# zcash-hackworks/bn

Measured on AMD Instinct MI355X. Metric: BN254 optimal-ate pairings/sec (bit-exact vs ref), higher is better.
Workload: dtype u32; 1 GPU; 2^16 independent pairings per step on 1 MI355X (BASELINE.json configs[1]); pairings_per_gpu=65536, inputs=r*G1 / s*G2 (Jacobian, z != 1) resident in HBM, parallelism=dp1 (sharded, no collective), mapping=1, cus=256, pairings_per_launch=65536

## Files before the change

### bn_amd/csrc/bn254_constants.hpp

```cpp
#pragma once
#include <stdint.h>
#ifndef BN254_CONSTANT
#define BN254_CONSTANT constexpr
#endif
namespace bn254 { namespace k {
constexpr int W = 29, N = 9;
BN254_CONSTANT uint32_t MASK = 0x1fffffffu;
BN254_CONSTANT uint32_t Q[9] = {0x187cfd47u, 0x010460b6u, 0x1c72a34fu, 0x02d522d0u, 0x1585d978u, 0x02db40c0u, 0x00a6e141u, 0x0e5c2634u, 0x0030644eu};
BN254_CONSTANT uint32_t QINV = 0x04866389u;
BN254_CONSTANT uint32_t FE_MU = 0xa948e8c4u;
BN254_CONSTANT uint32_t FE_MU24 = 0x00a948e8u;
BN254_CONSTANT uint32_t ONE[9] = {0x157ccc21u, 0x141c2758u, 0x185230d3u, 0x014c0419u, 0x0aa36fb9u, 0x1d4240ceu, 0x11d54c07u, 0x052ac7a8u, 0x000dc836u};
BN254_CONSTANT uint32_t C_IN[9] = {0x13349ca1u, 0x1a5d84a8u, 0x0a3e5cacu, 0x100249e0u, 0x12b951e8u, 0x0e92d304u, 0x14cb95b3u, 0x041b9d3du, 0x00058003u};
BN254_CONSTANT uint32_t C_OUT[9] = {0x058f0d9du, 0x1aea1c6eu, 0x11c2cf74u, 0x11d651ebu, 0x1462c0a7u, 0x11b7bc3cu, 0x1cbd99bau, 0x183340fbu, 0x000e0a77u};
BN254_CONSTANT uint32_t RAW_ONE[9] = {0x00000001u, 0x00000000u, 0x00000000u, 0x00000000u, 0x00000000u, 0x00000000u, 0x00000000u, 0x00000000u, 0x00000000u};
BN254_CONSTANT uint32_t TWO_INV[9] = {0x16fce4b4u, 0x0a904407u, 0x0a626a11u, 0x12109375u, 0x1014a498u, 0x100ec0c7u, 0x093e16a4u, 0x09c376eeu, 0x001f1642u};
BN254_CONSTANT uint32_t G2_B[2][9] = {{0x0b489658u, 0x00cfd255u, 0x0fdb9a77u, 0x02ce89f7u, 0x0033a0d4u, 0x1a768545u, 0x06ee3ddcu, 0x106a7dc1u, 0x0019316bu}, {0x1b9fece0u, 0x07ecccd1u, 0x1069f1c7u, 0x0cdf64f3u, 0x0154cbe1u, 0x0dd22ac0u, 0x06eba4e8u, 0x1929a235u, 0x00283739u}};
BN254_CONSTANT uint32_t G2_3B[2][9] = {{0x095cc5c1u, 0x016b1649u, 0x13202c16u, 0x05967b15u, 0x0b150904u, 0x0c884f0eu, 0x1423d855u, 0x02e3530fu, 0x001b2ff4u}, {0x01e5cc12u, 0x15bda508u, 0x18588eb7u, 0x00f3e938u, 0x18f2b0b4u, 0x03bffebeu, 0x13752c37u, 0x0ec49a37u, 0x0017dd10u}};
BN254_CONSTANT uint32_t ISO_T2[9] = {0x1e3bec37u, 0x007b2046u, 0x19d0ea1fu, 0x1acb991fu, 0x13795f5du, 0x1055c3f5u, 0x15c8f72cu, 0x101310f5u, 0x002bf6bau};
BN254_CONSTANT uint32_t ISO_T3[9] = {0x1af1f8a3u, 0x00cd9858u, 0x1dce6a34u, 0x142e620au, 0x1bc0c667u, 0x0ae94d20u, 0x0db9310bu, 0x12572b72u, 0x000405e6u};
BN254_CONSTANT uint32_t FROB6_C1[4][2][9] = {
    {{0x157ccc21u, 0x141c2758u, 0x185230d3u, 0x014c0419u, 0x0aa36fb9u, 0x1d4240ceu, 0x11d54c07u, 0x052ac7a8u, 0x000dc836u}, {0x00000000u, 0x00000000u, 0x00000000u, 0x00000000u, 0x00000000u, 0x00000000u, 0x00000000u, 0x00000000u, 0x00000000u}},
    {{0x04a59190u, 0x06f504d9u, 0x0bf870bbu, 0x171ffd5cu, 0x1ac4d17du, 0x04be36d5u, 0x0bceec27u, 0x1a83a513u, 0x002492b3u}, {0x11142ef1u, 0x0b31acc7u, 0x1d5818bcu, 0x180afc17u, 0x1a63177eu, 0x15765b3bu, 0x118f742eu, 0x063a509au, 0x00135e4eu}},
    {{0x18ccb791u, 0x175b1c3au, 0x0b83d6e2u, 0x0e8ed071u, 0x1282bee2u, 0x04220e84u, 0x1fe4017fu, 0x15084d4au, 0x00169119u}, {0x00000000u, 0x00000000u, 0x00000000u, 0x00000000u, 0x00000000u, 0x00000000u, 0x00000000u, 0x00000000u, 0x00000000u}},
// ... 27 lines not shown
BN254_CONSTANT uint32_t TWIST_MUL_BY_Q_X[2][9] = {{0x04a59190u, 0x06f504d9u, 0x0bf870bbu, 0x171ffd5cu, 0x1ac4d17du, 0x04be36d5u, 0x0bceec27u, 0x1a83a513u, 0x002492b3u}, {0x11142ef1u, 0x0b31acc7u, 0x1d5818bcu, 0x180afc17u, 0x1a63177eu, 0x15765b3bu, 0x118f742eu, 0x063a509au, 0x00135e4eu}};
BN254_CONSTANT uint32_t TWIST_MUL_BY_Q_Y[2][9] = {{0x1b1f0678u, 0x0373fb06u, 0x13170fbdu, 0x185d74b7u, 0x0241131fu, 0x16e18435u, 0x1ef3b6ceu, 0x01f06f02u, 0x001d46bdu}, {0x19a647d5u, 0x19fdefabu, 0x1d925d1au, 0x0d1f6c5fu, 0x08ac6cc5u, 0x1fa5621au, 0x134f06feu, 0x09a72816u, 0x0015871du}};
BN254_CONSTANT uint64_t ATE_LOOP_LOW64 = 0x9d797039be763ba8ull;
BN254_CONSTANT uint64_t BN_U = 0x44e992b44a6909f1ull;
constexpr int BN_U_NAF_LEN = 63;
BN254_CONSTANT int8_t BN_U_NAF[63] = {1, 0, 0, 0, -1, 0, 0, 0, 0, 1, 0, 1, 0, 0, 0, 0, 1, 0, 0, 1, 0, -1, 0, 1, 0, 1, 0, 1, 0, 0, 1, 0, 0, 0, 1, 0, -1, 0, -1, 0, -1, 0, 1, 0, 1, 0, 0, -1, 0, 1, 0, 1, 0, -1, 0, 0, 1, 0, 1, 0, 0, 0, 1};
constexpr int EXP_SLOTS = 9;
constexpr int EXP_STEPS = 63;
BN254_CONSTANT int32_t EXP_SCHED[63] = {64, 1, 1, 1, 131, 195, 1, 1, 1, 1, 1, 39, 1, 1, 1, 1, 1, 1, 5, 1, 7, 1, 1, 1, 39, 1, 1, 1, 39, 1, 1, 1, 1, 1, 1, 1, 1, 7, 1, 1, 1, 7, 1, 1, 1, 1, 1, 5, 1, 1, 1, 1, 7, 1, 1, 1, 1, 37, 1, 1, 1, 1, 16389};
constexpr int FE_STEPS = 204;
BN254_CONSTANT int32_t FE_PROG[204] = {256, 64, 1, 1, 1, 131, 195, 1, 1, 1, 1, 1, 39, 1, 1, 1, 1, 1, 1, 5, 1, 7, 1, 1, 1, 39, 1, 1, 1, 39, 1, 1, 1, 1, 1, 1, 1, 1, 7, 1, 1, 1, 7, 1, 1, 1, 1, 1, 5, 1, 1, 1, 1, 7, 1, 1, 1, 1, 37, 1, 1, 1, 1, 16389, 321, 395, 64, 1, 1, 1, 131, 195, 1, 1, 1, 1, 1, 39, 1, 1, 1, 1, 1, 1, 5, 1, 7, 1, 1, 1, 39, 1, 1, 1, 39, 1, 1, 1, 1, 1, 1, 1, 1, 7, 1, 1, 1, 7, 1, 1, 1, 1, 1, 5, 1, 1, 1, 1, 7, 1, 1, 1, 1, 37, 1, 1, 1, 1, 16837, 1, 64, 1, 1, 1, 131, 195, 1, 1, 1, 1, 1, 39, 1, 1, 1, 1, 1, 1, 5, 1, 7, 1, 1, 1, 39, 1, 1, 1, 39, 1, 1, 1, 1, 1, 1, 1, 1, 7, 1, 1, 1, 7, 1, 1, 1, 1, 1, 5, 1, 1, 1, 1, 7, 1, 1, 1, 1, 37, 1, 1, 1, 1, 5, 14, 556, 586, 8206, 392, 41984, 460, 57344, 334, 74792, 10};
constexpr int ATE_NAF_LEN = 66;
BN254_CONSTANT int8_t ATE_NAF[66] = {0, 0, 0, 1, 0, 1, 0, -1, 0, 0, -1, 0, 0, 0, 1, 0, 0, -1, 0, -1, 0, 0, 0, 1, 0, -1, 0, 0, 0, 0, -1, 0, 0, 1, 0, -1, 0, 0, 1, 0, 0, 0, 0, 0, -1, 0, 0, -1, 0, 1, 0, -1, 0, 0, 0, -1, 0, -1, 0, 0, 0, 1, 0, -1, 0, 1};
BN254_CONSTANT int32_t Q30[9] = {0x187cfd47, 0x3082305b, 0x071ca8d3, 0x205aa45a, 0x01585d97, 0x0116da06, 0x1a029b85, 0x139cb84c, 0x00003064};
BN254_CONSTANT uint32_t QINV30 = 0x1b799c77u;
BN254_CONSTANT uint32_t C_R3[9] = {0x0e2312b2u, 0x16c05ca2u, 0x0bc84389u, 0x1cdf310bu, 0x11adafddu, 0x032e568eu, 0x1d6ae48cu, 0x10d4cd1fu, 0x0026c2d2u};
BN254_CONSTANT uint32_t C_RAW_IN[9] = {0x059bac10u, 0x0d1503a3u, 0x018016b8u, 0x10ab0ca8u, 0x02632639u, 0x02c0169fu, 0x169bfd53u, 0x11869d4cu, 0x002a11a6u};
BN254_CONSTANT uint32_t C_RAW_HI[9] = {0x0ff8e86au, 0x07c648f0u, 0x0d256c51u, 0x0e144bb5u, 0x0fe5cb16u, 0x0e4726c0u, 0x07f5c538u, 0x0f6c68ccu, 0x00043c5bu};
BN254_CONSTANT uint32_t Q32[8] = {0xd87cfd47u, 0x3c208c16u, 0x6871ca8du, 0x97816a91u, 0x8181585du, 0xb85045b6u, 0xe131a029u, 0x30644e72u};
BN254_CONSTANT uint32_t QINV256[8] = {0x1b799c77u, 0x782df87du, 0xe1359536u, 0x6121829au, 0xe7cc257fu, 0x2750342fu, 0x6e777394u, 0x0a85dd48u};
BN254_CONSTANT uint64_t R_MINUS_1[4] = {0x43e1f593f0000000ull, 0x2833e84879b97091ull, 0xb85045b68181585dull, 0x30644e72e131a029ull};
BN254_CONSTANT uint32_t G1_B[9] = {0x00766463u, 0x1c54760au, 0x08f6927au, 0x03e40c4du, 0x1fea4f2bu, 0x17c6c26au, 0x157fe417u, 0x0f8056f9u, 0x002958a2u};
BN254_CONSTANT uint64_t Q_MINUS_2[4] = {0x3c208c16d87cfd45ull, 0x97816a916871ca8dull, 0xb85045b68181585dull, 0x30644e72e131a029ull};
BN254_CONSTANT uint32_t H2C_C2[9] = {0x01801893u, 0x16741cafu, 0x1210393du, 0x10c48f5bu, 0x057134dfu, 0x12cc7ff9u, 0x1768ca9cu, 0x0498af45u, 0x00114e0cu};
BN254_CONSTANT uint32_t H2C_C3[9] = {0x1b4a814fu, 0x1d686287u, 0x16a42cbau, 0x0bac1e79u, 0x013fb16cu, 0x1d850693u, 0x1eba05b6u, 0x0c9dae1eu, 0x001b5818u};
BN254_CONSTANT uint32_t H2C_C4[9] = {0x068a0e4bu, 0x171eba7cu, 0x0b55234fu, 0x150690b3u, 0x0ed0a792u, 0x1ff392cau, 0x026922c2u, 0x109d85a1u, 0x002768ebu};
BN254_CONSTANT uint32_t H2C_G2_C1[2][9] = {{0x00c56279u, 0x14ebf9aeu, 0x082dcb4au, 0x041a8e11u, 0x0ad7108du, 0x17b8c613u, 0x18c389e4u, 0x15954569u, 0x0026f9a1u}, {0x1b9fece0u, 0x07ecccd1u, 0x1069f1c7u, 0x0cdf64f3u, 0x0154cbe1u, 0x0dd22ac0u, 0x06eba4e8u, 0x1929a235u, 0x00283739u}};
BN254_CONSTANT uint32_t H2C_G2_C3[2][9] = {{0x1ac12654u, 0x18b51d52u, 0x02b71328u, 0x0f302745u, 0x18dae6dfu, 0x1ec740f3u, 0x0ad8391fu, 0x1e701b16u, 0x002bf9c5u}, {0x1b8c55e3u, 0x07029597u, 0x09a398b3u, 0x06a5295fu, 0x152a0cd2u, 0x1080d518u, 0x1295607fu, 0x1129d51au, 0x00151bebu}};
BN254_CONSTANT uint32_t H2C_G2_C4[2][9] = {{0x1a9d7742u, 0x1b78c9dau, 0x18a8378fu, 0x1586dd8au, 0x1c979cdeu, 0x1b6acebcu, 0x159e5ffbu, 0x15469a85u, 0x002cd11au}, {0x017a140eu, 0x0ccd05abu, 0x0dad5994u, 0x148069b2u, 0x09454dc3u, 0x089e4881u, 0x1813914cu, 0x05d61ecbu, 0x002b29a5u}};
BN254_CONSTANT uint32_t GLV_BETA[9] = {0x0a337995u, 0x158d1d23u, 0x189c9b98u, 0x12fa4e45u, 0x185faadcu, 0x0176f16du, 0x0eed93bau, 0x14291140u, 0x000c0afeu};
BN254_CONSTANT uint32_t GLV_G1[3] = {0xc7e0b3d7u, 0xd91d232eu, 0x00000002u};
// ... 17 lines not shown
```

### bn_amd/csrc/fe.hpp

```cpp
#pragma once
#include <stdint.h>

#if defined(BN_HOSTSIM)
#define BN_FN inline
#define BN_LEAF inline
#define BN_LEAF_MUL inline
#define BN_LEAF_RED inline
#define BN_COARSE inline
#define BN_OUTER inline
#define BN254_CONSTANT constexpr
#define BN_COMPILER_FENCE() ((void)0)
#else
#include <hip/hip_runtime.h>
#define BN_FN __device__ __forceinline__
#define BN_LEAF __device__ __noinline__ inline
#ifdef BN_INLINE_ALL
#define BN_LEAF_MUL __device__ __forceinline__
#define BN_LEAF_RED __device__ __forceinline__
#define BN_COARSE __device__ __forceinline__
#else
#define BN_LEAF_MUL BN_LEAF
#define BN_LEAF_RED BN_LEAF
#define BN_COARSE __device__ __noinline__ inline
#endif
// ... 883 lines not shown
    uint32_t u = 1, v = 0, q = 0, r = 1, f = f0, g = g0;
#pragma unroll 1
    for (int i = 0; i < 30; ++i) {
        uint32_t mask1 = (uint32_t)(zeta >> 31);
        uint32_t mask2 = 0u - (g & 1u);
        uint32_t x = (f ^ mask1) - mask1, y = (u ^ mask1) - mask1, z = (v ^ mask1) - mask1;
        g += x & mask2; q += y & mask2; r += z & mask2;
        mask1 &= mask2;
        zeta = (int32_t)((uint32_t)zeta ^ mask1) - 1;
        f += g & mask1; u += q & mask1; v += r & mask1;
        g >>= 1; u <<= 1; v <<= 1;
    }
    tu = (int32_t)u; tv = (int32_t)v; tq = (int32_t)q; tr = (int32_t)r;
    return zeta;
}
BN_FN void divsteps_update_de(Signed30 &d, Signed30 &e, int32_t u, int32_t v, int32_t q, int32_t r) {
    const int32_t M30 = 0x3fffffff;
    int32_t sd = d.v[8] >> 31, se = e.v[8] >> 31;
    int32_t md = (u & sd) + (v & se), me = (q & sd) + (r & se);
    int32_t di = d.v[0], ei = e.v[0];
    int64_t cd = (int64_t)u * di + (int64_t)v * ei, ce = (int64_t)q * di + (int64_t)r * ei;
    md -= (int32_t)((k::QINV30 * (uint32_t)cd + (uint32_t)md) & (uint32_t)M30);
    me -= (int32_t)((k::QINV30 * (uint32_t)ce + (uint32_t)me) & (uint32_t)M30);
    cd += (int64_t)k::Q30[0] * md;
    ce += (int64_t)k::Q30[0] * me;
    cd >>= 30; ce >>= 30;
#pragma unroll
    for (int i = 1; i < 9; ++i) {
        di = d.v[i]; ei = e.v[i];
        cd += (int64_t)u * di + (int64_t)v * ei + (int64_t)k::Q30[i] * md;
// ... 18 lines not shown
    }
    f.v[8] = (int32_t)cf; g.v[8] = (int32_t)cg;
}
BN_FN Fe fe_inverse_body(const Fe &a_in) {
    BN_REQUIRE(a_in.lb <= 2 && a_in.vb <= 8 && !a_in.sg, "fe_inverse input");
    uint32_t w[8];
    fe_pack_u32x8(fe_canonical(fe_mul(a_in, fe_const(k::ONE))), w);
    Signed30 f, g, d, e;
#pragma unroll
    for (int i = 0; i < 9; ++i) {
        int bit = 30 * i, wi = bit >> 5, sh = bit & 31;
        uint64_t two = (uint64_t)w[wi] | (wi + 1 < 8 ? ((uint64_t)w[wi + 1] << 32) : 0);
        g.v[i] = (int32_t)((uint32_t)(two >> sh) & 0x3fffffffu);
        f.v[i] = k::Q30[i];
        d.v[i] = 0;
        e.v[i] = i == 0 ? 1 : 0;
    }
    int32_t zeta = -1;
#pragma unroll 1
    for (int it = 0; it < 20; ++it) {
        int32_t tu, tv, tq, tr;
        zeta = divsteps_30(zeta, (uint32_t)f.v[0], (uint32_t)g.v[0], tu, tv, tq, tr);
        divsteps_update_de(d, e, tu, tv, tq, tr);
        divsteps_update_fg(f, g, tu, tv, tq, tr);
    }
    const int32_t M30 = 0x3fffffff;
    int32_t r[9];
    int32_t cond_add = d.v[8] >> 31, cond_neg = f.v[8] >> 31;
#pragma unroll
    for (int i = 0; i < 9; ++i) { int32_t t = d.v[i] + (k::Q30[i] & cond_add); r[i] = (t ^ cond_neg) - cond_neg; }
#pragma unroll
    for (int i = 0; i < 8; ++i) { r[i + 1] += r[i] >> 30; r[i] &= M30; }
    cond_add = r[8] >> 31;
#pragma unroll
    for (int i = 0; i < 9; ++i) r[i] += k::Q30[i] & cond_add;
#pragma unroll
    for (int i = 0; i < 8; ++i) { r[i + 1] += r[i] >> 30; r[i] &= M30; }
#pragma unroll
    for (int j = 0; j < 8; ++j) {
        int bit = 32 * j, li = bit / 30, sh = bit - 30 * li;
        uint64_t vv = (uint64_t)(uint32_t)r[li] >> sh;
        if (li + 1 < 9) vv |= (uint64_t)(uint32_t)r[li + 1] << (30 - sh);
        w[j] = (uint32_t)vv;
    }
    return fe_mul(fe_unpack_u32x8(w), fe_const(k::C_R3));
}
BN_LEAF1(fe_inverse, fe_inverse_body)

}
```

### bn_amd/csrc/fe_asm.hpp

```cpp
#pragma once
namespace bn254 {
BN_FN Fe fe_mul_asm(const Fe &a, const Fe &b) {
    uint64_t acc;
    uint32_t m[9];
    Fe r;
    asm("v_mad_u64_u32 %0, vcc, %1, %2, 0" : "=&v"(acc) : "v"(a.l[0]), "v"(b.l[0]) : "vcc");
    m[0] = ((uint32_t)acc * k::QINV) & MASK29; acc += (uint64_t)m[0] * k::Q[0]; acc >>= 29;
    asm("v_mad_u64_u32 %0, vcc, %1, %2, %0\n\tv_mad_u64_u32 %0, vcc, %3, %4, %0\n\tv_mad_u64_u32 %0, vcc, %5, %6, %0" : "+v"(acc) : "v"(a.l[0]), "v"(b.l[1]), "v"(a.l[1]), "v"(b.l[0]), "v"(m[0]), "s"(k::Q[1]) : "vcc");
    m[1] = ((uint32_t)acc * k::QINV) & MASK29; acc += (uint64_t)m[1] * k::Q[0]; acc >>= 29;
    asm("v_mad_u64_u32 %0, vcc, %1, %2, %0\n\tv_mad_u64_u32 %0, vcc, %3, %4, %0\n\tv_mad_u64_u32 %0, vcc, %5, %6, %0\n\tv_mad_u64_u32 %0, vcc, %7, %8, %0\n\tv_mad_u64_u32 %0, vcc, %9, %10, %0" : "+v"(acc) : "v"(a.l[0]), "v"(b.l[2]), "v"(a.l[1]), "v"(b.l[1]), "v"(a.l[2]), "v"(b.l[0]), "v"(m[0]), "s"(k::Q[2]), "v"(m[1]), "s"(k::Q[1]) : "vcc");
    m[2] = ((uint32_t)acc * k::QINV) & MASK29; acc += (uint64_t)m[2] * k::Q[0]; acc >>= 29;
    asm("v_mad_u64_u32 %0, vcc, %1, %2, %0\n\tv_mad_u64_u32 %0, vcc, %3, %4, %0\n\tv_mad_u64_u32 %0, vcc, %5, %6, %0\n\tv_mad_u64_u32 %0, vcc, %7, %8, %0\n\tv_mad_u64_u32 %0, vcc, %9, %10, %0\n\tv_mad_u64_u32 %0, vcc, %11, %12, %0\n\tv_mad_u64_u32 %0, vcc, %13, %14, %0" : "+v"(acc) : "v"(a.l[0]), "v"(b.l[3]), "v"(a.l[1]), "v"(b.l[2]), "v"(a.l[2]), "v"(b.l[1]), "v"(a.l[3]), "v"(b.l[0]), "v"(m[0]), "s"(k::Q[3]), "v"(m[1]), "s"(k::Q[2]), "v"(m[2]), "s"(k::Q[1]) : "vcc");
    m[3] = ((uint32_t)acc * k::QINV) & MASK29; acc += (uint64_t)m[3] * k::Q[0]; acc >>= 29;
    asm("v_mad_u64_u32 %0, vcc, %1, %2, %0\n\tv_mad_u64_u32 %0, vcc, %3, %4, %0\n\tv_mad_u64_u32 %0, vcc, %5, %6, %0\n\tv_mad_u64_u32 %0, vcc, %7, %8, %0\n\tv_mad_u64_u32 %0, vcc, %9, %10, %0\n\tv_mad_u64_u32 %0, vcc, %11, %12, %0\n\tv_mad_u64_u32 %0, vcc, %13, %14, %0\n\tv_mad_u64_u32 %0, vcc, %15, %16, %0\n\tv_mad_u64_u32 %0, vcc, %17, %18, %0" : "+v"(acc) : "v"(a.l[0]), "v"(b.l[4]), "v"(a.l[1]), "v"(b.l[3]), "v"(a.l[2]), "v"(b.l[2]), "v"(a.l[3]), "v"(b.l[1]), "v"(a.l[4]), "v"(b.l[0]), "v"(m[0]), "s"(k::Q[4]), "v"(m[1]), "s"(k::Q[3]), "v"(m[2]), "s"(k::Q[2]), "v"(m[3]), "s"(k::Q[1]) : "vcc");
    m[4] = ((uint32_t)acc * k::QINV) & MASK29; acc += (uint64_t)m[4] * k::Q[0]; acc >>= 29;
    asm("v_mad_u64_u32 %0, vcc, %1, %2, %0\n\tv_mad_u64_u32 %0, vcc, %3, %4, %0\n\tv_mad_u64_u32 %0, vcc, %5, %6, %0\n\tv_mad_u64_u32 %0, vcc, %7, %8, %0\n\tv_mad_u64_u32 %0, vcc, %9, %10, %0\n\tv_mad_u64_u32 %0, vcc, %11, %12, %0\n\tv_mad_u64_u32 %0, vcc, %13, %14, %0\n\tv_mad_u64_u32 %0, vcc, %15, %16, %0\n\tv_mad_u64_u32 %0, vcc, %17, %18, %0\n\tv_mad_u64_u32 %0, vcc, %19, %20, %0\n\tv_mad_u64_u32 %0, vcc, %21, %22, %0" : "+v"(acc) : "v"(a.l[0]), "v"(b.l[5]), "v"(a.l[1]), "v"(b.l[4]), "v"(a.l[2]), "v"(b.l[3]), "v"(a.l[3]), "v"(b.l[2]), "v"(a.l[4]), "v"(b.l[1]), "v"(a.l[5]), "v"(b.l[0]), "v"(m[0]), "s"(k::Q[5]), "v"(m[1]), "s"(k::Q[4]), "v"(m[2]), "s"(k::Q[3]), "v"(m[3]), "s"(k::Q[2]), "v"(m[4]), "s"(k::Q[1]) : "vcc");
    m[5] = ((uint32_t)acc * k::QINV) & MASK29; acc += (uint64_t)m[5] * k::Q[0]; acc >>= 29;
    asm("v_mad_u64_u32 %0, vcc, %1, %2, %0\n\tv_mad_u64_u32 %0, vcc, %3, %4, %0\n\tv_mad_u64_u32 %0, vcc, %5, %6, %0\n\tv_mad_u64_u32 %0, vcc, %7, %8, %0\n\tv_mad_u64_u32 %0, vcc, %9, %10, %0\n\tv_mad_u64_u32 %0, vcc, %11, %12, %0\n\tv_mad_u64_u32 %0, vcc, %13, %14, %0\n\tv_mad_u64_u32 %0, vcc, %15, %16, %0\n\tv_mad_u64_u32 %0, vcc, %17, %18, %0\n\tv_mad_u64_u32 %0, vcc, %19, %20, %0\n\tv_mad_u64_u32 %0, vcc, %21, %22, %0\n\tv_mad_u64_u32 %0, vcc, %23, %24, %0\n\tv_mad_u64_u32 %0, vcc, %25, %26, %0" : "+v"(acc) : "v"(a.l[0]), "v"(b.l[6]), "v"(a.l[1]), "v"(b.l[5]), "v"(a.l[2]), "v"(b.l[4]), "v"(a.l[3]), "v"(b.l[3]), "v"(a.l[4]), "v"(b.l[2]), "v"(a.l[5]), "v"(b.l[1]), "v"(a.l[6]), "v"(b.l[0]), "v"(m[0]), "s"(k::Q[6]), "v"(m[1]), "s"(k::Q[5]), "v"(m[2]), "s"(k::Q[4]), "v"(m[3]), "s"(k::Q[3]), "v"(m[4]), "s"(k::Q[2]), "v"(m[5]), "s"(k::Q[1]) : "vcc");
    m[6] = ((uint32_t)acc * k::QINV) & MASK29; acc += (uint64_t)m[6] * k::Q[0]; acc >>= 29;
    asm("v_mad_u64_u32 %0, vcc, %1, %2, %0\n\tv_mad_u64_u32 %0, vcc, %3, %4, %0\n\tv_mad_u64_u32 %0, vcc, %5, %6, %0\n\tv_mad_u64_u32 %0, vcc, %7, %8, %0\n\tv_mad_u64_u32 %0, vcc, %9, %10, %0\n\tv_mad_u64_u32 %0, vcc, %11, %12, %0\n\tv_mad_u64_u32 %0, vcc, %13, %14, %0\n\tv_mad_u64_u32 %0, vcc, %15, %16, %0\n\tv_mad_u64_u32 %0, vcc, %17, %18, %0\n\tv_mad_u64_u32 %0, vcc, %19, %20, %0\n\tv_mad_u64_u32 %0, vcc, %21, %22, %0\n\tv_mad_u64_u32 %0, vcc, %23, %24, %0\n\tv_mad_u64_u32 %0, vcc, %25, %26, %0\n\tv_mad_u64_u32 %0, vcc, %27, %28, %0\n\tv_mad_u64_u32 %0, vcc, %29, %30, %0" : "+v"(acc) : "v"(a.l[0]), "v"(b.l[7]), "v"(a.l[1]), "v"(b.l[6]), "v"(a.l[2]), "v"(b.l[5]), "v"(a.l[3]), "v"(b.l[4]), "v"(a.l[4]), "v"(b.l[3]), "v"(a.l[5]), "v"(b.l[2]), "v"(a.l[6]), "v"(b.l[1]), "v"(a.l[7]), "v"(b.l[0]), "v"(m[0]), "s"(k::Q[7]), "v"(m[1]), "s"(k::Q[6]), "v"(m[2]), "s"(k::Q[5]), "v"(m[3]), "s"(k::Q[4]), "v"(m[4]), "s"(k::Q[3]), "v"(m[5]), "s"(k::Q[2]), "v"(m[6]), "s"(k::Q[1]) : "vcc");
    m[7] = ((uint32_t)acc * k::QINV) & MASK29; acc += (uint64_t)m[7] * k::Q[0]; acc >>= 29;
    asm("v_mad_u64_u32 %0, vcc, %1, %2, %0\n\tv_mad_u64_u32 %0, vcc, %3, %4, %0\n\tv_mad_u64_u32 %0, vcc, %5, %6, %0\n\tv_mad_u64_u32 %0, vcc, %7, %8, %0\n\tv_mad_u64_u32 %0, vcc, %9, %10, %0\n\tv_mad_u64_u32 %0, vcc, %11, %12, %0\n\tv_mad_u64_u32 %0, vcc, %13, %14, %0\n\tv_mad_u64_u32 %0, vcc, %15, %16, %0\n\tv_mad_u64_u32 %0, vcc, %17, %18, %0\n\tv_mad_u64_u32 %0, vcc, %19, %20, %0\n\tv_mad_u64_u32 %0, vcc, %21, %22, %0\n\tv_mad_u64_u32 %0, vcc, %23, %24, %0\n\tv_mad_u64_u32 %0, vcc, %25, %26, %0\n\tv_mad_u64_u32 %0, vcc, %27, %28, %0\n\tv_mad_u64_u32 %0, vcc, %29, %30, %0\n\tv_mad_u64_u32 %0, vcc, %31, %32, %0\n\tv_mad_u64_u32 %0, vcc, %33, %34, %0" : "+v"(acc) : "v"(a.l[0]), "v"(b.l[8]), "v"(a.l[1]), "v"(b.l[7]), "v"(a.l[2]), "v"(b.l[6]), "v"(a.l[3]), "v"(b.l[5]), "v"(a.l[4]), "v"(b.l[4]), "v"(a.l[5]), "v"(b.l[3]), "v"(a.l[6]), "v"(b.l[2]), "v"(a.l[7]), "v"(b.l[1]), "v"(a.l[8]), "v"(b.l[0]), "v"(m[0]), "s"(k::Q[8]), "v"(m[1]), "s"(k::Q[7]), "v"(m[2]), "s"(k::Q[6]), "v"(m[3]), "s"(k::Q[5]), "v"(m[4]), "s"(k::Q[4]), "v"(m[5]), "s"(k::Q[3]), "v"(m[6]), "s"(k::Q[2]), "v"(m[7]), "s"(k::Q[1]) : "vcc");
    m[8] = ((uint32_t)acc * k::QINV) & MASK29; acc += (uint64_t)m[8] * k::Q[0]; acc >>= 29;
    asm("v_mad_u64_u32 %0, vcc, %1, %2, %0\n\tv_mad_u64_u32 %0, vcc, %3, %4, %0\n\tv_mad_u64_u32 %0, vcc, %5, %6, %0\n\tv_mad_u64_u32 %0, vcc, %7, %8, %0\n\tv_mad_u64_u32 %0, vcc, %9, %10, %0\n\tv_mad_u64_u32 %0, vcc, %11, %12, %0\n\tv_mad_u64_u32 %0, vcc, %13, %14, %0\n\tv_mad_u64_u32 %0, vcc, %15, %16, %0\n\tv_mad_u64_u32 %0, vcc, %17, %18, %0\n\tv_mad_u64_u32 %0, vcc, %19, %20, %0\n\tv_mad_u64_u32 %0, vcc, %21, %22, %0\n\tv_mad_u64_u32 %0, vcc, %23, %24, %0\n\tv_mad_u64_u32 %0, vcc, %25, %26, %0\n\tv_mad_u64_u32 %0, vcc, %27, %28, %0\n\tv_mad_u64_u32 %0, vcc, %29, %30, %0\n\tv_mad_u64_u32 %0, vcc, %31, %32, %0" : "+v"(acc) : "v"(a.l[1]), "v"(b.l[8]), "v"(a.l[2]), "v"(b.l[7]), "v"(a.l[3]), "v"(b.l[6]), "v"(a.l[4]), "v"(b.l[5]), "v"(a.l[5]), "v"(b.l[4]), "v"(a.l[6]), "v"(b.l[3]), "v"(a.l[7]), "v"(b.l[2]), "v"(a.l[8]), "v"(b.l[1]), "v"(m[1]), "s"(k::Q[8]), "v"(m[2]), "s"(k::Q[7]), "v"(m[3]), "s"(k::Q[6]), "v"(m[4]), "s"(k::Q[5]), "v"(m[5]), "s"(k::Q[4]), "v"(m[6]), "s"(k::Q[3]), "v"(m[7]), "s"(k::Q[2]), "v"(m[8]), "s"(k::Q[1]) : "vcc");
// ... 459 lines not shown
    r.l[2] = (uint32_t)acc & MASK29; acc = (uint64_t)((int64_t)acc >> 29);
    asm("v_mad_u64_u32 %0, vcc, 1, %1, %0\n\tv_mad_i64_i32 %0, vcc, 9, %2, %0\n\tv_mad_i64_i32 %0, vcc, %3, %4, %0\n\tv_mad_u64_u32 %0, vcc, %5, %6, %0\n\tv_mad_u64_u32 %0, vcc, %7, %8, %0\n\tv_mad_u64_u32 %0, vcc, %9, %10, %0\n\tv_mad_u64_u32 %0, vcc, %11, %12, %0\n\tv_mad_u64_u32 %0, vcc, %13, %14, %0\n\tv_mad_i64_i32 %0, vcc, %15, %16, %0\n\tv_mad_i64_i32 %0, vcc, -1, %17, %0" : "+v"(acc) : "v"(n.l[12]), "v"(x.l[12]), "v"(s), "v"(px.l[12]), "v"(m[4]), "s"(k::Q[8]), "v"(m[5]), "s"(k::Q[7]), "v"(m[6]), "s"(k::Q[6]), "v"(m[7]), "s"(k::Q[5]), "v"(m[8]), "s"(k::Q[4]), "v"(kq), "s"(-(int32_t)k::Q[3]), "v"(d.l[3]) : "vcc");
    r.l[3] = (uint32_t)acc & MASK29; acc = (uint64_t)((int64_t)acc >> 29);
    asm("v_mad_u64_u32 %0, vcc, 1, %1, %0\n\tv_mad_i64_i32 %0, vcc, 9, %2, %0\n\tv_mad_i64_i32 %0, vcc, %3, %4, %0\n\tv_mad_u64_u32 %0, vcc, %5, %6, %0\n\tv_mad_u64_u32 %0, vcc, %7, %8, %0\n\tv_mad_u64_u32 %0, vcc, %9, %10, %0\n\tv_mad_u64_u32 %0, vcc, %11, %12, %0\n\tv_mad_i64_i32 %0, vcc, %13, %14, %0\n\tv_mad_i64_i32 %0, vcc, -1, %15, %0" : "+v"(acc) : "v"(n.l[13]), "v"(x.l[13]), "v"(s), "v"(px.l[13]), "v"(m[5]), "s"(k::Q[8]), "v"(m[6]), "s"(k::Q[7]), "v"(m[7]), "s"(k::Q[6]), "v"(m[8]), "s"(k::Q[5]), "v"(kq), "s"(-(int32_t)k::Q[4]), "v"(d.l[4]) : "vcc");
    r.l[4] = (uint32_t)acc & MASK29; acc = (uint64_t)((int64_t)acc >> 29);
    asm("v_mad_u64_u32 %0, vcc, 1, %1, %0\n\tv_mad_i64_i32 %0, vcc, 9, %2, %0\n\tv_mad_i64_i32 %0, vcc, %3, %4, %0\n\tv_mad_u64_u32 %0, vcc, %5, %6, %0\n\tv_mad_u64_u32 %0, vcc, %7, %8, %0\n\tv_mad_u64_u32 %0, vcc, %9, %10, %0\n\tv_mad_i64_i32 %0, vcc, %11, %12, %0\n\tv_mad_i64_i32 %0, vcc, -1, %13, %0" : "+v"(acc) : "v"(n.l[14]), "v"(x.l[14]), "v"(s), "v"(px.l[14]), "v"(m[6]), "s"(k::Q[8]), "v"(m[7]), "s"(k::Q[7]), "v"(m[8]), "s"(k::Q[6]), "v"(kq), "s"(-(int32_t)k::Q[5]), "v"(d.l[5]) : "vcc");
    r.l[5] = (uint32_t)acc & MASK29; acc = (uint64_t)((int64_t)acc >> 29);
    asm("v_mad_u64_u32 %0, vcc, 1, %1, %0\n\tv_mad_i64_i32 %0, vcc, 9, %2, %0\n\tv_mad_i64_i32 %0, vcc, %3, %4, %0\n\tv_mad_u64_u32 %0, vcc, %5, %6, %0\n\tv_mad_u64_u32 %0, vcc, %7, %8, %0\n\tv_mad_i64_i32 %0, vcc, %9, %10, %0\n\tv_mad_i64_i32 %0, vcc, -1, %11, %0" : "+v"(acc) : "v"(n.l[15]), "v"(x.l[15]), "v"(s), "v"(px.l[15]), "v"(m[7]), "s"(k::Q[8]), "v"(m[8]), "s"(k::Q[7]), "v"(kq), "s"(-(int32_t)k::Q[6]), "v"(d.l[6]) : "vcc");
    r.l[6] = (uint32_t)acc & MASK29; acc = (uint64_t)((int64_t)acc >> 29);
    asm("v_mad_u64_u32 %0, vcc, 1, %1, %0\n\tv_mad_i64_i32 %0, vcc, 9, %2, %0\n\tv_mad_i64_i32 %0, vcc, %3, %4, %0\n\tv_mad_u64_u32 %0, vcc, %5, %6, %0\n\tv_mad_i64_i32 %0, vcc, %7, %8, %0\n\tv_mad_i64_i32 %0, vcc, -1, %9, %0" : "+v"(acc) : "v"(n.l[16]), "v"(x.l[16]), "v"(s), "v"(px.l[16]), "v"(m[8]), "s"(k::Q[8]), "v"(kq), "s"(-(int32_t)k::Q[7]), "v"(d.l[7]) : "vcc");
    r.l[7] = (uint32_t)acc & MASK29; acc = (uint64_t)((int64_t)acc >> 29);
    asm("v_mad_i64_i32 %0, vcc, 1, %1, %0\n\tv_mad_i64_i32 %0, vcc, 9, %2, %0\n\tv_mad_i64_i32 %0, vcc, %3, %4, %0\n\tv_mad_i64_i32 %0, vcc, %5, %6, %0\n\tv_mad_i64_i32 %0, vcc, -1, %7, %0" : "+v"(acc) : "v"(n.l[17]), "v"(x.l[17]), "v"(s), "v"(px.l[17]), "v"(kq), "s"(-(int32_t)k::Q[8]), "v"(d.l[8]) : "vcc");
    r.l[8] = (uint32_t)acc;
    return r;
}
}
```

### bn_amd/csrc/pairing.hpp

```cpp
#pragma once
#include "tower.hpp"

namespace bn254 {

template <class F2> struct G2Proj { F2 x, y, z; };
template <class F2> struct G2Aff { F2 x, y; };
template <class S> struct G1Aff { S x, y; };
template <class F2> struct Line { F2 ell_0, ell_vw, ell_vv; };

#define F2P ((const F2 *)nullptr)

template <bool ISO = false, class F2>
BN_COARSE Line<F2> doubling_step(G2Proj<F2> &r) {
    F2 a = f2_half(f2_mul(r.x, r.y));
    F2 b = f2_sqr(r.y), c = f2_sqr(r.z);
    F2 e;
    if constexpr (ISO) e = f2_mul_iso3b(c);
    else e = f2_mul_const(c, k::G2_3B);
    F2 f3 = f2_add(f2_add(e, e), e);
    F2 g = f2_half_for_sqr(f2_add(b, f3));
    F2 h = f2_lc3<1, -1, -1>(f2_sqr(f2_sum_for_mul(r.y, r.z)), b, c);
    F2 j = f2_sqr(r.x), e_sq = f2_sqr(e);
    Line<F2> l;
    l.ell_0 = f2_mul_xi(f2_ssub(e, b));
    l.ell_vw = f2_neg_lazy(h);
    l.ell_vv = f2_add(f2_add(j, j), j);
    r.x = f2_mul(a, f2_lc3<1, -3, 0>(b, e, e));
    r.y = f2_lc3<1, -3, 0>(f2_sqr(g), e_sq, e_sq);
// ... 62 lines not shown
        int digit = 1;
        if (!tail) {
            if (NAF) digit = k::ATE_NAF[ND - 1 - j];
            else digit = (int)((k::ATE_LOOP_LOW64 >> (63 - (j & 63))) & 1);
        }
        if (j == ND) st.put_base(mul_by_q(st.get_base()));
        if (j == ND + 1) { G2Aff<F2> b2 = mul_by_q(st.get_base()); b2.y = f2_neg(b2.y); st.put_base(b2); }
#pragma unroll 1
        for (int pass = tail ? 1 : 0; pass < (digit != 0 ? 2 : 1); ++pass) {
            BN_MILLER_HOOK(2 * j + pass, 2 * (ND + 2));
            Line<F2> l;
            if (pass == 0) {
                if (j != 0) f = f12_sqr(f);
                BN_COMPILER_FENCE();
                G2Proj<F2> r = st.get_r();
                l = doubling_step<NAF>(r);
                st.put_r(r);
            } else {
                G2Proj<F2> r = st.get_r();
                G2Aff<F2> b = st.get_base();
                if (NAF && digit < 0) b.y = f2_neg(b.y);
                l = addition_step(r, b);
                st.put_r(r);
            }
            f = apply_line(f, l, st.get_p());
        }
    }
    return f;
}
template <int M, class F2, class S, class Store>
BN_FN Fq12<F2> miller_loop_shared(Store &st) {
// ... 9 lines not shown
                G2Aff<F2> b = mul_by_q(st.get_base(i));
                if (j == ND + 1) b.y = f2_neg(b.y);
                st.put_base(i, b);
            }
        }
#pragma unroll 1
        for (int pass = tail ? 1 : 0; pass < (digit != 0 ? 2 : 1); ++pass) {
            BN_MILLER_HOOK(2 * j + pass, 2 * (ND + 2));
            if (pass == 0 && j != 0) f = f12_sqr(f);
#pragma unroll 1
            for (int i = 0; i < M; ++i) {
                BN_COMPILER_FENCE();
                G2Proj<F2> r = st.get_r(i);
                Line<F2> l;
                if (pass == 0) {
                    l = doubling_step<true>(r);
                } else {
                    G2Aff<F2> b = st.get_base(i);
                    if (digit < 0) b.y = f2_neg(b.y);
                    l = addition_step(r, b);
                }
                st.put_r(i, r);
                const G1Aff<S> p = st.get_p(i);
                F2 x0 = l.ell_0, x4 = f2_scale(l.ell_vw, p.y), x2 = f2_scale(l.ell_vv, p.x);
                const bool inf = st.is_inf(i);
                x0 = f2_select(inf, x0, f2_one(F2P)); x4 = f2_select(inf, x4, f2_zero(F2P)); x2 = f2_select(inf, x2, f2_zero(F2P));
                f = f12_mul_by_024(f, x0, x4, x2);
            }
        }
    }
    return f;
// ... 65 lines not shown
    const S t2 = f2_scalar_const(F2P, k::ISO_T2), t3 = f2_scalar_const(F2P, k::ISO_T3);
    G2Aff<F2> base = {f2_scale(q_in.x, t2), f2_scale(q_in.y, t3)};
    G2Proj<F2> r = {base.x, base.y, f2_one(F2P)};
    F2 pref = f2_one(F2P);
    int idx = 0;
#pragma unroll 1
    for (int j = 0; j < ND + 2; ++j) {
        const bool tail = j >= ND;
        const int digit = tail ? 1 : k::ATE_NAF[ND - 1 - j];
        if (j == ND) base = mul_by_q(base);
        if (j == ND + 1) { base = mul_by_q(base); base.y = f2_neg(base.y); }
#pragma unroll 1
        for (int pass = tail ? 1 : 0; pass < (digit != 0 ? 2 : 1); ++pass) {
            Line<F2> l;
            if (pass == 0) {
                l = doubling_step<true>(r);
            } else {
                G2Aff<F2> b = base;
                if (digit < 0) b.y = f2_neg(b.y);
                l = addition_step(r, b);
            }
            const F2 d = f2_scale(l.ell_vw, t3), c = f2_scale(l.ell_vv, t2);
            pref = f2_mul(pref, d);
            st.put_raw(idx, l.ell_0, d, c, pref);
            ++idx;
        }
    }
    F2 inv = f2_inverse(pref);
#pragma unroll 1
    for (idx = NATIVE_LINES - 1; idx >= 0; --idx) {
        F2 e0, d, c;
// ... 264 lines not shown
```

Measured before the change: 10.23 million pairings/s.

## Use squaring-based doubling, asm divsteps, and fold inverse correction into initial e

Adds a squaring-based G2 doubling step in which products are formed as squares of sums, and makes it the default in the Miller loops and in precompute. Replaces the divsteps inner loop in the field inverse with an inline GCN assembly version that uses bfi and xad, and folds the final Montgomery R^3 correction into a precomputed starting value of e, which removes one fe_mul per inversion. These are separate micro-optimisations aimed at VALU instruction count. The scaled doubling changes the projective representation (the outputs are scaled by 2 or 4) and the line coefficients, which relies on the final exponentiation to cancel the scaling. The handwritten asm bypasses compiler scheduling.

```diff
diff --git a/bn_amd/csrc/bn254_constants.hpp b/bn_amd/csrc/bn254_constants.hpp
--- a/bn_amd/csrc/bn254_constants.hpp
+++ b/bn_amd/csrc/bn254_constants.hpp
@@ -65,7 +65,7 @@
 BN254_CONSTANT int8_t ATE_NAF[66] = {0, 0, 0, 1, 0, 1, 0, -1, 0, 0, -1, 0, 0, 0, 1, 0, 0, -1, 0, -1, 0, 0, 0, 1, 0, -1, 0, 0, 0, 0, -1, 0, 0, 1, 0, -1, 0, 0, 1, 0, 0, 0, 0, 0, -1, 0, 0, -1, 0, 1, 0, -1, 0, 0, 0, -1, 0, -1, 0, 0, 0, 1, 0, -1, 0, 1};
 BN254_CONSTANT int32_t Q30[9] = {0x187cfd47, 0x3082305b, 0x071ca8d3, 0x205aa45a, 0x01585d97, 0x0116da06, 0x1a029b85, 0x139cb84c, 0x00003064};
 BN254_CONSTANT uint32_t QINV30 = 0x1b799c77u;
-BN254_CONSTANT uint32_t C_R3[9] = {0x0e2312b2u, 0x16c05ca2u, 0x0bc84389u, 0x1cdf310bu, 0x11adafddu, 0x032e568eu, 0x1d6ae48cu, 0x10d4cd1fu, 0x0026c2d2u};
+BN254_CONSTANT int32_t INV_E0_30[9] = {0x259bac10, 0x068a81d1, 0x006005ae, 0x26156195, 0x3e263263, 0x131600b4, 0x265a6ff5, 0x29a30d3a, 0x00002a11};
 BN254_CONSTANT uint32_t C_RAW_IN[9] = {0x059bac10u, 0x0d1503a3u, 0x018016b8u, 0x10ab0ca8u, 0x02632639u, 0x02c0169fu, 0x169bfd53u, 0x11869d4cu, 0x002a11a6u};
 BN254_CONSTANT uint32_t C_RAW_HI[9] = {0x0ff8e86au, 0x07c648f0u, 0x0d256c51u, 0x0e144bb5u, 0x0fe5cb16u, 0x0e4726c0u, 0x07f5c538u, 0x0f6c68ccu, 0x00043c5bu};
 BN254_CONSTANT uint32_t Q32[8] = {0xd87cfd47u, 0x3c208c16u, 0x6871ca8du, 0x97816a91u, 0x8181585du, 0xb85045b6u, 0xe131a029u, 0x30644e72u};
diff --git a/bn_amd/csrc/fe.hpp b/bn_amd/csrc/fe.hpp
--- a/bn_amd/csrc/fe.hpp
+++ b/bn_amd/csrc/fe.hpp
@@ -921,6 +921,22 @@
     tu = (int32_t)u; tv = (int32_t)v; tq = (int32_t)q; tr = (int32_t)r;
     return zeta;
 }
+BN_FN int32_t divsteps_30_fused(int32_t zeta, uint32_t f0, uint32_t g0, int32_t &tu, int32_t &tv, int32_t &tq, int32_t &tr) {
+    uint32_t u = 1, v = 0, q = 0, r = 1, f = f0, g = g0, x;
+    for (int i = 0; i < 30; ++i) {
+        const uint32_t m2 = (uint32_t)((int32_t)(g << 31) >> 31);
+        const uint32_t m1 = (uint32_t)(zeta >> 31);
+        const uint32_t s1 = (uint32_t)zeta >> 31;
+        const uint32_t sw = m1 & m2;
+        x = ((f ^ m1) + s1) & m2; f = (sw & g) | (~sw & f); g += x;
+        x = ((u ^ m1) + s1) & m2; u = (sw & q) | (~sw & u); q += x;
+        x = ((v ^ m1) + s1) & m2; v = (sw & r) | (~sw & v); r += x;
+        zeta = (int32_t)(((uint32_t)zeta ^ sw) + 0xffffffffu);
+        g >>= 1; u <<= 1; v <<= 1;
+    }
+    tu = (int32_t)u; tv = (int32_t)v; tq = (int32_t)q; tr = (int32_t)r;
+    return zeta;
+}
 BN_FN void divsteps_update_de(Signed30 &d, Signed30 &e, int32_t u, int32_t v, int32_t q, int32_t r) {
     const int32_t M30 = 0x3fffffff;
     int32_t sd = d.v[8] >> 31, se = e.v[8] >> 31;
@@ -969,13 +985,17 @@
         g.v[i] = (int32_t)((uint32_t)(two >> sh) & 0x3fffffffu);
         f.v[i] = k::Q30[i];
         d.v[i] = 0;
-        e.v[i] = i == 0 ? 1 : 0;
+        e.v[i] = k::INV_E0_30[i];
     }
     int32_t zeta = -1;
 #pragma unroll 1
     for (int it = 0; it < 20; ++it) {
         int32_t tu, tv, tq, tr;
+#if !defined(BN_HOSTSIM)
+        zeta = divsteps_30_asm(zeta, (uint32_t)f.v[0], (uint32_t)g.v[0], tu, tv, tq, tr);
+#else
         zeta = divsteps_30(zeta, (uint32_t)f.v[0], (uint32_t)g.v[0], tu, tv, tq, tr);
+#endif
         divsteps_update_de(d, e, tu, tv, tq, tr);
         divsteps_update_fg(f, g, tu, tv, tq, tr);
     }
@@ -998,7 +1018,7 @@
         if (li + 1 < 9) vv |= (uint64_t)(uint32_t)r[li + 1] << (30 - sh);
         w[j] = (uint32_t)vv;
     }
-    return fe_mul(fe_unpack_u32x8(w), fe_const(k::C_R3));
+    return fe_unpack_u32x8(w);
 }
 BN_LEAF1(fe_inverse, fe_inverse_body)
 
diff --git a/bn_amd/csrc/fe_asm.hpp b/bn_amd/csrc/fe_asm.hpp
--- a/bn_amd/csrc/fe_asm.hpp
+++ b/bn_amd/csrc/fe_asm.hpp
@@ -497,4 +497,13 @@
     r.l[8] = (uint32_t)acc;
     return r;
 }
-}
+BN_FN int32_t divsteps_30_asm(int32_t zeta, uint32_t f, uint32_t g, int32_t &tu, int32_t &tv, int32_t &tq, int32_t &tr) {
+    uint32_t u = 1, v = 0, q = 0, r = 1, m1, m2, s1, sw, x;
+#pragma unroll 1
+    for (int i = 0; i < 6; ++i)
+        asm("v_bfe_i32 %[m2], %[g], 0, 1\n\tv_ashrrev_i32 %[m1], 31, %[z]\n\tv_lshrrev_b32 %[s1], 31, %[z]\n\tv_and_b32 %[sw], %[m1], %[m2]\n\tv_xad_u32 %[x], %[f], %[m1], %[s1]\n\tv_and_b32 %[x], %[x], %[m2]\n\tv_bfi_b32 %[f], %[sw], %[g], %[f]\n\tv_add_u32 %[g], %[g], %[x]\n\tv_xad_u32 %[x], %[u], %[m1], %[s1]\n\tv_and_b32 %[x], %[x], %[m2]\n\tv_bfi_b32 %[u], %[sw], %[q], %[u]\n\tv_add_u32 %[q], %[q], %[x]\n\tv_xad_u32 %[x], %[v], %[m1], %[s1]\n\tv_and_b32 %[x], %[x], %[m2]\n\tv_bfi_b32 %[v], %[sw], %[r], %[v]\n\tv_add_u32 %[r], %[r], %[x]\n\tv_xad_u32 %[z], %[z], %[sw], -1\n\tv_lshrrev_b32 %[g], 1, %[g]\n\tv_lshlrev_b32 %[u], 1, %[u]\n\tv_lshlrev_b32 %[v], 1, %[v]\n\tv_bfe_i32 %[m2], %[g], 0, 1\n\tv_ashrrev_i32 %[m1], 31, %[z]\n\tv_lshrrev_b32 %[s1], 31, %[z]\n\tv_and_b32 %[sw], %[m1], %[m2]\n\tv_xad_u32 %[x], %[f], %[m1], %[s1]\n\tv_and_b32 %[x], %[x], %[m2]\n\tv_bfi_b32 %[f], %[sw], %[g], %[f]\n\tv_add_u32 %[g], %[g], %[x]\n\tv_xad_u32 %[x], %[u], %[m1], %[s1]\n\tv_and_b32 %[x], %[x], %[m2]\n\tv_bfi_b32 %[u], %[sw], %[q], %[u]\n\tv_add_u32 %[q], %[q], %[x]\n\tv_xad_u32 %[x], %[v], %[m1], %[s1]\n\tv_and_b32 %[x], %[x], %[m2]\n\tv_bfi_b32 %[v], %[sw], %[r], %[v]\n\tv_add_u32 %[r], %[r], %[x]\n\tv_xad_u32 %[z], %[z], %[sw], -1\n\tv_lshrrev_b32 %[g], 1, %[g]\n\tv_lshlrev_b32 %[u], 1, %[u]\n\tv_lshlrev_b32 %[v], 1, %[v]\n\tv_bfe_i32 %[m2], %[g], 0, 1\n\tv_ashrrev_i32 %[m1], 31, %[z]\n\tv_lshrrev_b32 %[s1], 31, %[z]\n\tv_and_b32 %[sw], %[m1], %[m2]\n\tv_xad_u32 %[x], %[f], %[m1], %[s1]\n\tv_and_b32 %[x], %[x], %[m2]\n\tv_bfi_b32 %[f], %[sw], %[g], %[f]\n\tv_add_u32 %[g], %[g], %[x]\n\tv_xad_u32 %[x], %[u], %[m1], %[s1]\n\tv_and_b32 %[x], %[x], %[m2]\n\tv_bfi_b32 %[u], %[sw], %[q], %[u]\n\tv_add_u32 %[q], %[q], %[x]\n\tv_xad_u32 %[x], %[v], %[m1], %[s1]\n\tv_and_b32 %[x], %[x], %[m2]\n\tv_bfi_b32 %[v], %[sw], %[r], %[v]\n\tv_add_u32 %[r], %[r], %[x]\n\tv_xad_u32 %[z], %[z], %[sw], -1\n\tv_lshrrev_b32 %[g], 1, %[g]\n\tv_lshlrev_b32 %[u], 1, %[u]\n\tv_lshlrev_b32 %[v], 1, %[v]\n\tv_bfe_i32 %[m2], %[g], 0, 1\n\tv_ashrrev_i32 %[m1], 31, %[z]\n\tv_lshrrev_b32 %[s1], 31, %[z]\n\tv_and_b32 %[sw], %[m1], %[m2]\n\tv_xad_u32 %[x], %[f], %[m1], %[s1]\n\tv_and_b32 %[x], %[x], %[m2]\n\tv_bfi_b32 %[f], %[sw], %[g], %[f]\n\tv_add_u32 %[g], %[g], %[x]\n\tv_xad_u32 %[x], %[u], %[m1], %[s1]\n\tv_and_b32 %[x], %[x], %[m2]\n\tv_bfi_b32 %[u], %[sw], %[q], %[u]\n\tv_add_u32 %[q], %[q], %[x]\n\tv_xad_u32 %[x], %[v], %[m1], %[s1]\n\tv_and_b32 %[x], %[x], %[m2]\n\tv_bfi_b32 %[v], %[sw], %[r], %[v]\n\tv_add_u32 %[r], %[r], %[x]\n\tv_xad_u32 %[z], %[z], %[sw], -1\n\tv_lshrrev_b32 %[g], 1, %[g]\n\tv_lshlrev_b32 %[u], 1, %[u]\n\tv_lshlrev_b32 %[v], 1, %[v]\n\tv_bfe_i32 %[m2], %[g], 0, 1\n\tv_ashrrev_i32 %[m1], 31, %[z]\n\tv_lshrrev_b32 %[s1], 31, %[z]\n\tv_and_b32 %[sw], %[m1], %[m2]\n\tv_xad_u32 %[x], %[f], %[m1], %[s1]\n\tv_and_b32 %[x], %[x], %[m2]\n\tv_bfi_b32 %[f], %[sw], %[g], %[f]\n\tv_add_u32 %[g], %[g], %[x]\n\tv_xad_u32 %[x], %[u], %[m1], %[s1]\n\tv_and_b32 %[x], %[x], %[m2]\n\tv_bfi_b32 %[u], %[sw], %[q], %[u]\n\tv_add_u32 %[q], %[q], %[x]\n\tv_xad_u32 %[x], %[v], %[m1], %[s1]\n\tv_and_b32 %[x], %[x], %[m2]\n\tv_bfi_b32 %[v], %[sw], %[r], %[v]\n\tv_add_u32 %[r], %[r], %[x]\n\tv_xad_u32 %[z], %[z], %[sw], -1\n\tv_lshrrev_b32 %[g], 1, %[g]\n\tv_lshlrev_b32 %[u], 1, %[u]\n\tv_lshlrev_b32 %[v], 1, %[v]"
+            : [z] "+v"(zeta), [f] "+v"(f), [g] "+v"(g), [u] "+v"(u), [v] "+v"(v), [q] "+v"(q), [r] "+v"(r), [m1] "=&v"(m1), [m2] "=&v"(m2), [s1] "=&v"(s1), [sw] "=&v"(sw), [x] "=&v"(x));
+    tu = (int32_t)u; tv = (int32_t)v; tq = (int32_t)q; tr = (int32_t)r;
+    return zeta;
+}
+}
diff --git a/bn_amd/csrc/pairing.hpp b/bn_amd/csrc/pairing.hpp
--- a/bn_amd/csrc/pairing.hpp
+++ b/bn_amd/csrc/pairing.hpp
@@ -10,8 +10,30 @@
 
 #define F2P ((const F2 *)nullptr)
 
-template <bool ISO = false, class F2>
+#ifndef BN254_DOUBLING_QUAD
+#define BN254_DOUBLING_QUAD 1
+#endif
+template <bool ISO = false, bool QUAD = false, class F2>
 BN_COARSE Line<F2> doubling_step(G2Proj<F2> &r) {
+    if constexpr (QUAD) {
+        F2 b = f2_sqr(r.y), c = f2_sqr(r.z), j = f2_sqr(r.x);
+        F2 a2 = f2_lc3<1, -1, -1>(f2_sqr(f2_sum_for_mul(r.x, r.y)), j, b);
+        F2 e;
+        if constexpr (ISO) e = f2_mul_iso3b(c);
+        else e = f2_mul_const(c, k::G2_3B);
+        F2 yz = f2_sqr(f2_sum_for_mul(r.y, r.z));
+        F2 h2 = f2_lc3<2, 0, 0>(f2_ssub(yz, f2_add(b, c)), yz, yz);
+        F2 e_sq = f2_sqr(e);
+        F2 j3 = f2_add(f2_add(j, j), j);
+        Line<F2> l;
+        l.ell_0 = f2_lc_xi<2, 0>(f2_ssub(e, b), b);
+        l.ell_vw = f2_neg_lazy(h2);
+        l.ell_vv = f2_add(j3, j3);
+        r.x = f2_mul(a2, f2_lc3<1, -3, 0>(b, e, e));
+        r.y = f2_lc3<1, -12, 0>(f2_sqr(f2_lc3<1, 3, 0>(b, e, e)), e_sq, e_sq);
+        r.z = f2_mul(f2_dbl(b), h2);
+        return l;
+    }
     F2 a = f2_half(f2_mul(r.x, r.y));
     F2 b = f2_sqr(r.y), c = f2_sqr(r.z);
     F2 e;
@@ -104,7 +126,7 @@
                 if (j != 0) f = f12_sqr(f);
                 BN_COMPILER_FENCE();
                 G2Proj<F2> r = st.get_r();
-                l = doubling_step<NAF>(r);
+                l = doubling_step<NAF, NAF && BN254_DOUBLING_QUAD != 0>(r);
                 st.put_r(r);
             } else {
                 G2Proj<F2> r = st.get_r();
@@ -144,7 +166,7 @@
                 G2Proj<F2> r = st.get_r(i);
                 Line<F2> l;
                 if (pass == 0) {
-                    l = doubling_step<true>(r);
+                    l = doubling_step<true, BN254_DOUBLING_QUAD != 0>(r);
                 } else {
                     G2Aff<F2> b = st.get_base(i);
                     if (digit < 0) b.y = f2_neg(b.y);
@@ -240,7 +262,7 @@
         for (int pass = tail ? 1 : 0; pass < (digit != 0 ? 2 : 1); ++pass) {
             Line<F2> l;
             if (pass == 0) {
-                l = doubling_step<true>(r);
+                l = doubling_step<true, BN254_DOUBLING_QUAD != 0>(r);
             } else {
                 G2Aff<F2> b = base;
                 if (digit < 0) b.y = f2_neg(b.y);
```

Measured after the change: 10.28 million pairings/s (median of 6 runs). About the same (+0.5%).
